# turbocast/HTS-train-WORLD

Measured on AMD Instinct MI355X. Metric: WORLD analysis+synthesis frames/sec @16kHz, 5ms hop, higher is better.
Workload: dtype f64

## Files before the change

### hts-train-world_amd/csrc/synthesis.hip

```cpp
#include <stdlib.h>

#include <algorithm>
#include <vector>

#include "batch.hpp"
#include "common.hpp"
#include "fastmath.hpp"
#include "fft.hpp"
#include "partition.hpp"

namespace wm {

__device__ __forceinline__ double coarse_f0(const double* __restrict__ f0, int nf, int j, double lowest) {
  if (j < nf) {
    const double v = f0[j];
    return v < lowest ? 0.0 : v;
  }
  const int j2 = nf >= 2 ? nf - 2 : nf - 1;
  const double a = f0[nf - 1] < lowest ? 0.0 : f0[nf - 1];
  const double b = f0[j2] < lowest ? 0.0 : f0[j2];
  return a * 2 - b;
}
__device__ __forceinline__ double coarse_vuv(const double* __restrict__ f0, int nf, int j, double lowest) {
  if (j < nf) return (f0[j] < lowest ? 0.0 : f0[j]) == 0.0 ? 0.0 : 1.0;
  const double a = (f0[nf - 1] < lowest ? 0.0 : f0[nf - 1]) == 0.0 ? 0.0 : 1.0;
  const int j2 = nf >= 2 ? nf - 2 : nf - 1;
  const double b = (f0[j2] < lowest ? 0.0 : f0[j2]) == 0.0 ? 0.0 : 1.0;
  return a * 2 - b;
}

#define WM_CHAIN_PRIO __builtin_amdgcn_s_setprio(3);
__global__ __launch_bounds__(256) void synth_inc_kernel(
    const int* __restrict__ utts, const double* __restrict__ f0, const int64_t* __restrict__ f_off,
    const int64_t* __restrict__ y_off, int fs, double fp, double lowest_f0, double* __restrict__ vuv_out,
    double* __restrict__ inc_out) {
#pragma clang fp contract(off)
  WM_CHAIN_PRIO
  const int u = utts[blockIdx.y];
  const double* f0u = f0 + f_off[u];
  const int nf = (int)(f_off[u + 1] - f_off[u]);
  const int64_t yb = y_off[u];
  const int ylen = (int)(y_off[u + 1] - yb);
  for (int i = blockIdx.x * 256 + threadIdx.x; i < ylen; i += gridDim.x * 256) {
    const double t = i / (double)fs;
    int kg = (int)(t / fp) + 1;
    if (kg > nf + 1) kg = nf + 1;
    if (kg < 0) kg = 0;
    while (kg <= nf && kg * fp <= t) ++kg;
    while (kg > 0 && (kg - 1) * fp > t) --kg;
    const int k = kg < 1 ? 1 : (kg > nf ? nf : kg);
    const double x0 = (k - 1) * fp, x1 = k * fp;
    const double h = x1 - x0;
    const double s = (t - x0) / h;
    const double fa = coarse_f0(f0u, nf, k - 1, lowest_f0), fb = coarse_f0(f0u, nf, k, lowest_f0);
    const double va = coarse_vuv(f0u, nf, k - 1, lowest_f0), vb = coarse_vuv(f0u, nf, k, lowest_f0);
    double fi = fa + s * (fb - fa);
    const double vi = va + s * (vb - va);
    const double vv = vi > 0.5 ? 1.0 : 0.0;
    fi = vv == 0.0 ? kDefaultF0 : fi;
    vuv_out[yb + i] = vv;
    inc_out[yb + i] = 2.0 * kPi * fi / fs;
  }
}

__global__ __launch_bounds__(64) void synth_timebase_kernel(const int* __restrict__ utts,
                                                            const int64_t* __restrict__ y_off, double* phase) {
#pragma clang fp contract(off)
  WM_CHAIN_PRIO
  const int u = utts[blockIdx.x], lane = threadIdx.x;
  const int64_t yb = y_off[u];
  const int ylen = (int)(y_off[u + 1] - yb);
  double carry = 0.0;
  constexpr int kSuper = 1024, kPer = kSuper / 64;
  __shared__ double ring[2 * kSuper];
  const double* p = phase + yb;
  double stage[kPer];
  auto request = [&](int s0) {
#pragma unroll
    for (int q = 0; q < kPer; ++q) {
      const int idx = s0 + 64 * q + lane;
      stage[q] = p[imin(idx, ylen - 1)];
    }
  };
  auto park = [&](int half) {
#pragma unroll
    for (int q = 0; q < kPer; ++q) ring[half * kSuper + 64 * q + lane] = stage[q];
  };
  request(0);
  park(0);
  request(kSuper);
  __syncthreads();
  double r[16];
#pragma unroll
  for (int q = 0; q < 16; ++q) r[q] = ring[q];
  for (int c0 = 0; c0 < ylen; c0 += 64) {
    const int i = c0 + lane;
    if ((c0 & (kSuper - 1)) == 0) {
      park(((c0 / kSuper) + 1) & 1);
      request(c0 + 2 * kSuper);
      __syncthreads();
    }
    double t = carry;
#pragma unroll
    for (int g = 0; g < 4; ++g) {
      double n[16];
      const int nb = (c0 + 16 * (g + 1)) & (2 * kSuper - 1);
#pragma unroll
      for (int q = 0; q < 16; ++q) n[q] = ring[nb + q];
#define WM_STEP(R) "v_add_f64 %[t], %[t], %[" #R "]\n\ts_lshl_b64 exec, exec, 1\n\t"
      asm volatile(
          "s_lshl_b64 exec, -1, %[sh]\n\t"
          WM_STEP(b0) WM_STEP(b1) WM_STEP(b2) WM_STEP(b3) WM_STEP(b4) WM_STEP(b5) WM_STEP(b6) WM_STEP(b7)
          WM_STEP(b8) WM_STEP(b9) WM_STEP(b10) WM_STEP(b11) WM_STEP(b12) WM_STEP(b13) WM_STEP(b14)
          "v_add_f64 %[t], %[t], %[b15]\n\t"
          "s_mov_b64 exec, -1"
          : [t] "+v"(t)
          : [sh] "n"(16 * g), [b0] "v"(r[0]), [b1] "v"(r[1]), [b2] "v"(r[2]), [b3] "v"(r[3]), [b4] "v"(r[4]),
            [b5] "v"(r[5]), [b6] "v"(r[6]), [b7] "v"(r[7]), [b8] "v"(r[8]), [b9] "v"(r[9]), [b10] "v"(r[10]),
            [b11] "v"(r[11]), [b12] "v"(r[12]), [b13] "v"(r[13]), [b14] "v"(r[14]), [b15] "v"(r[15])
          : "scc");
#undef WM_STEP
#pragma unroll
      for (int q = 0; q < 16; ++q) r[q] = n[q];
    }
    if (i < ylen) phase[yb + i] = t;
    carry = lane63(t);
  }
}

__device__ __forceinline__ double wrap_two_pi(double t) {
  const double two_pi = 2.0 * kPi;
  const double a = fabs(t);
  double kq = floor(a * (1.0 / two_pi));
  double w = __fma_rn(-kq, two_pi, a);
  if (w < 0.0) { kq -= 1.0; w = __fma_rn(-kq, two_pi, a); }
  if (w >= two_pi) { kq += 1.0; w = __fma_rn(-kq, two_pi, a); }
  return copysign(w, t);
}

constexpr int kSearchSub = 8, kSearchTile = 256 * kSearchSub;
template <bool WRITE>
__global__ __launch_bounds__(256) void synth_pulse_search_kernel(
    const int* __restrict__ utts, const int64_t* __restrict__ y_off, const double* __restrict__ phase, int fs,
    int tiles_max, int* __restrict__ tile_cnt, int* __restrict__ pulse_idx, double* __restrict__ pulse_shift,
    int* __restrict__ pulse_cnt) {
#pragma clang fp contract(off)
  WM_CHAIN_PRIO
  __shared__ int wave_cnt[kSearchSub][4];
  __shared__ int red[4];
  const int u = utts[blockIdx.y], tile = blockIdx.x;
  const int lane = threadIdx.x & 63, wv = threadIdx.x >> 6;
  const int64_t yb = y_off[u];
  const int ylen = (int)(y_off[u + 1] - yb);
  const int i0 = tile * kSearchTile;
  if (i0 >= ylen && !(WRITE && tile == 0)) return;
  int* cnt_u = tile_cnt + (int64_t)u * tiles_max;
  int count = 0;
  if (WRITE) {
    const int ntile = (ylen + kSearchTile - 1) / kSearchTile;
    int before = 0, all = 0;
    for (int j = threadIdx.x; j < ntile; j += 256) {
      const int c = cnt_u[j];
      all += c;
      if (j < tile) before += c;
    }
    before = wave_sum_i(before);
    all = wave_sum_i(all);
    if (lane == 0) red[wv] = before;
    __syncthreads();
    count = red[0] + red[1] + red[2] + red[3];
    __syncthreads();
    if (tile == 0) {
      if (lane == 0) red[wv] = all;
      __syncthreads();
      if (threadIdx.x == 0) pulse_cnt[u] = red[0] + red[1] + red[2] + red[3];
      __syncthreads();
    }
    if (i0 >= ylen) return;
  }
  double tc[kSearchSub], tp[kSearchSub];
#pragma unroll
  for (int q = 0; q < kSearchSub; ++q) {
    const int i = i0 + 256 * q + threadIdx.x;
    const bool in = i >= 1 && i < ylen;
    tc[q] = phase[yb + (in ? i : 0)];
    tp[q] = phase[yb + (in ? i - 1 : 0)];
  }
  bool hit[kSearchSub];
  double wrap[kSearchSub], prev[kSearchSub];
  unsigned long long bal[kSearchSub];
#pragma unroll
  for (int q = 0; q < kSearchSub; ++q) {
    const int i = i0 + 256 * q + threadIdx.x;
    wrap[q] = wrap_two_pi(tc[q]);
    prev[q] = wrap_two_pi(tp[q]);
    hit[q] = i >= 1 && i < ylen && fabs(wrap[q] - prev[q]) > kPi;
    bal[q] = __ballot(hit[q]);
    if (lane == 0) wave_cnt[q][wv] = __popcll(bal[q]);
  }
  __syncthreads();
  if (!WRITE) {
    if (threadIdx.x == 0) {
      int c = 0;
#pragma unroll
      for (int q = 0; q < kSearchSub; ++q) c += wave_cnt[q][0] + wave_cnt[q][1] + wave_cnt[q][2] + wave_cnt[q][3];
      cnt_u[tile] = c;
    }
    return;
  }
#pragma unroll
  for (int q = 0; q < kSearchSub; ++q) {
    const int i = i0 + 256 * q + threadIdx.x;
    int base = count;
    for (int w = 0; w < wv; ++w) base += wave_cnt[q][w];
    if (hit[q]) {
      const int dst = base + __popcll(bal[q] & ((1ull << lane) - 1ull));
      const double y1 = prev[q] - 2.0 * kPi, y2 = wrap[q];
      const double xx = -y1 / (y2 - y1);
      pulse_idx[yb + dst] = i - 1;
      pulse_shift[yb + dst] = xx / fs;
    }
    count += wave_cnt[q][0] + wave_cnt[q][1] + wave_cnt[q][2] + wave_cnt[q][3];
  }
}

__global__ __launch_bounds__(256) void synth_pulse_off_kernel(const int* __restrict__ utts, const int* __restrict__ cnt,
                                                              int n_list, int64_t base, int64_t* __restrict__ off,
                                                              int64_t* __restrict__ info) {
  __shared__ int64_t part[256];
  __shared__ int mx[256];
  const int per = (n_list + 255) / 256;
  const int lo = threadIdx.x * per, hi = imin(n_list, lo + per);
  int64_t sum = 0;
  int m = 0;
  for (int k = lo; k < hi; ++k) {
    const int c = cnt[utts[k]];
    sum += c;
    m = imax(m, c);
  }
  part[threadIdx.x] = sum;
  mx[threadIdx.x] = m;
  __syncthreads();
  if (threadIdx.x == 0) {
    int64_t run = 0;
    int mm = 0;
    for (int i = 0; i < 256; ++i) {
      const int64_t v = part[i];
      part[i] = run;
      run += v;
      mm = imax(mm, mx[i]);
    }
    info[0] = run;
    info[1] = mm;
    __threadfence_system();
  }
  __syncthreads();
  int64_t run = base + part[threadIdx.x];
  for (int k = lo; k < hi; ++k) {
    const int u = utts[k];
    off[u] = run;
    run += cnt[u];
  }
}

__global__ void synth_dc_remover_kernel(int fft_size, double* __restrict__ dcr) {
  if (threadIdx.x != 0 || blockIdx.x != 0) return;
  double dc = 0.0;
  const int h = fft_size / 2;
  for (int i = 0; i < h; ++i) {
    dcr[i] = 0.5 - 0.5 * cos(2.0 * kPi * (i + 1.0) / (1.0 + fft_size));
    dcr[fft_size - i - 1] = dcr[i];
    dc += dcr[i] * 2.0;
  }
  for (int i = 0; i < h; ++i) {
    dcr[i] /= dc;
    dcr[fft_size - i - 1] = dcr[i];
  }
}

__device__ __forceinline__ double safe_ap(double v) {
  const double m = 0.999999999999 < v ? 0.999999999999 : v;
  return 0.001 > m ? 0.001 : m;
}

template <int N>
__device__ __forceinline__ void minimum_phase(const double* ls, cpx* img, const FftTw<N>& tw, int lane,
                                              cpx (&mp)[N / 64 + 1]) {
  constexpr int M = N / 64, F = 2 * N, H = N;
  lane = opaque_lane(lane);
  cpx v[M];
#pragma unroll
  for (int m = 0; m < M; ++m) {
    const int i0 = 2 * (lane + 64 * m), i1 = i0 + 1;
    v[m] = make_double2(ls[i0 <= H ? i0 : F - i0], ls[i1 <= H ? i1 : F - i1]);
  }
  rfft_forward<N>(v, img, img, tw, lane);
#pragma unroll
  for (int m = 0; m < M; ++m) {
    const int i0 = 2 * (lane + 64 * m), i1 = i0 + 1;
    const double xa = img[imin(i0, H)].x, xb = img[imin(i1, H)].x;
    const double a = i0 <= H ? ((i0 == 0 || i0 == H) ? xa : 2.0 * xa) : 0.0;
    const double b = i1 < H ? 2.0 * xb : 0.0;
    v[m] = make_double2(a, b);
  }
  rfft_forward<N>(v, img, img, tw, lane);
#pragma unroll
  for (int m = 0; m <= M; ++m) {
    const int k = m < M ? lane + 64 * m : N;
    const cpx s = img[k];
    const double amp = wm_exp(s.x / F);
    double sn, cs;
    if (m < M) {
      sincospi(s.y * (1.0 / (kPi * F)), &sn, &cs);
    } else {
      sn = 0.0;
      cs = 1.0;
    }
    mp[m] = make_double2(amp * cs, amp * sn);
    __builtin_amdgcn_sched_barrier(0);
  }
  wave_sync();
}

template <int N>
__device__ __forceinline__ void minimum_phase_pair(const double* lsp, const double* lsa, cpx* img, const FftTw<N>& tw,
                                                   int lane, double (&php)[N / 64], double (&pha)[N / 64]) {
  constexpr int M = N / 64, F = 2 * N, H = N;
  static_assert(M >= 8 && M % 8 == 0, "the constant factors below are eighths of a half turn");
  lane = opaque_lane(lane);
  cpx v[M];
#pragma unroll
  for (int m = 0; m < M; ++m) {
    const int i0 = 2 * (lane + 64 * m), i1 = i0 + 1;
    const int a0 = i0 <= H ? i0 : F - i0, a1 = i1 <= H ? i1 : F - i1;
    const double p0 = lsp[a0], q0 = lsa[a0], p1 = lsp[a1], q1 = lsa[a1];
    v[m] = make_double2(p0 - q1, q0 + p1);
  }
  fft_forward<N>(v, img, tw, lane);
  auto turn = [&](int m, cpx e0, cpx& e, double& inv) {
    const int k64 = 32 * m / M;
    e = k64 % 16 == 0 ? e0 : cmul(e0, cconj(cis64(k64 % 16)));
    if (k64 / 16 == 1) e = make_double2(-e.y, e.x);
    const double r0 = __builtin_amdgcn_rcp(e.y);
    const double r1 = __builtin_fma(__builtin_fma(-e.y, r0, 1.0), r0, r0);
    inv = (m == 0 && lane == 0) ? 0.0 : 0.5 * r1;
  };
  wave_sync();
#pragma unroll
  for (int m = 0; m < M; ++m) img[lane + 64 * m] = v[m];
  wave_sync();
  {
    const cpx e0 = cconj(make_double2(opaque_d(tw.wsplit.x), opaque_d(tw.wsplit.y)));
    cpx zp[M];
#pragma unroll
    for (int m = 0; m < M; ++m) zp[m] = img[(N - (lane + 64 * m)) & (N - 1)];
    wave_sync();
#pragma unroll
    for (int m = 0; m < M; ++m) {
      cpx e;
      double inv;
      turn(m, e0, e, inv);
      const cpx R = make_double2((zp[m].x - v[m].x) * inv, (zp[m].y - v[m].y) * inv);
      const double ax = v[m].x + __builtin_fma(e.x, R.y, e.y * R.x) + R.x;
      const double ay = v[m].y - __builtin_fma(e.x, R.x, -(e.y * R.y)) + R.y;
      const cpx g = (m == 0 && lane == 0) ? make_double2(0.0, 0.0) : make_double2(2.0 * ax, 2.0 * ay);
      img[lane + 64 * m] = g;
      __builtin_amdgcn_sched_barrier(0);
    }
    if (lane == 0) img[H] = make_double2(0.0, 0.0);
  }
  wave_sync();
#pragma unroll
  for (int m = 0; m < M; ++m) {
    const int i0 = 2 * (lane + 64 * m), i1 = i0 + 1;
    const cpx c0 = img[i0 <= H ? i0 : F - i0], c1 = img[i1 <= H ? i1 : F - i1];
    const double s0 = i0 <= H ? 1.0 : -1.0, s1 = i1 <= H ? 1.0 : -1.0;
    v[m] = make_double2(s0 * c0.x - s1 * c1.y, s0 * c0.y + s1 * c1.x);
  }
  fft_forward<N>(v, img, tw, lane);
  wave_sync();
#pragma unroll
  for (int m = 0; m < M; ++m) img[lane + 64 * m] = v[m];
  wave_sync();
  {
    const cpx e0 = cconj(make_double2(opaque_d(tw.wsplit.x), opaque_d(tw.wsplit.y)));
#pragma unroll
    for (int m = 0; m < M; ++m) {
      const int k = lane + 64 * m;
      const cpx zp = img[(N - k) & (N - 1)];
      cpx e;
      double inv;
      turn(m, e0, e, inv);
      const cpx R = make_double2(-(zp.x + v[m].x) * inv, -(zp.y + v[m].y) * inv);
      const double gx = v[m].x + __builtin_fma(e.x, R.y, e.y * R.x) + R.x;
      const double gy = v[m].y - __builtin_fma(e.x, R.x, -(e.y * R.y)) + R.y;
      const bool zero = m == 0 && lane == 0;
      php[m] = zero ? 0.0 : gy * (0.5 / F);
      pha[m] = zero ? 0.0 : -gx * (0.5 / F);
      __builtin_amdgcn_sched_barrier(0);
    }
  }
  wave_sync();
}

struct PulseRec {
  int64_t fbase;
  int nf;
  int idx;
  int roff;
  int noise_size;
  double shift;
  double cvuv;
};

struct PulseVoicedPred {
  const PulseRec* rec;
  __device__ bool operator()(int i) const { return rec[i].cvuv > 0.5; }
};

constexpr int kOlaStep = 128;
__host__ __device__ inline int64_t ola_table_base(int64_t yb, int u) { return yb / kOlaStep + 2 * (int64_t)u; }

__global__ __launch_bounds__(256) void synth_pulse_rec_kernel(
    const int* __restrict__ utts, const int64_t* __restrict__ f_off, const int64_t* __restrict__ y_off,
    const int64_t* __restrict__ p_off, const int* __restrict__ p_cnt, const int* __restrict__ pulse_idx,
    const double* __restrict__ pulse_shift, const double* __restrict__ vuv, PulseRec* __restrict__ rec,
    int* __restrict__ first) {
  const int u = utts[blockIdx.y];
  const int64_t pb = p_off[u];
  const int np = p_cnt[u];
  const int64_t yb = y_off[u];
  const int ylen = (int)(y_off[u + 1] - yb);
  int* fu = first + ola_table_base(yb, u);
  const int m_last = (ylen + kOlaStep - 1) / kOlaStep;
  for (int pi = blockIdx.x * 256 + threadIdx.x; pi < np; pi += gridDim.x * 256) {
    PulseRec r;
    r.fbase = f_off[u];
    r.nf = (int)(f_off[u + 1] - f_off[u]);
    r.idx = pulse_idx[yb + pi];
    r.roff = r.idx - pulse_idx[yb];
    r.noise_size = pulse_idx[yb + imin(np - 1, pi + 1)] - r.idx;
    r.shift = pulse_shift[yb + pi];
    r.cvuv = vuv[yb + r.idx];
    rec[pb + pi] = r;
    const int prev = pi > 0 ? pulse_idx[yb + pi - 1] : -1;
    for (int m = prev < 0 ? 0 : prev / kOlaStep + 1; m <= imin(m_last, r.idx / kOlaStep); ++m) fu[m] = pi;
    if (pi == np - 1)
      for (int m = r.idx / kOlaStep + 1; m <= m_last; ++m) fu[m] = np;
  }
}

template <int F>
__global__ __launch_bounds__(64, F >= 4096 ? 1 : (F == 1024 ? 4 : (F < 1024 ? 3 : 2))) void synth_pulse_kernel(
    const double* __restrict__ sp, const double* __restrict__ ap, const PulseRec* __restrict__ rec,
    const double* __restrict__ dcr, const uint32_t* __restrict__ rtab, int fs, double fp, int64_t p_begin,
    int64_t p_end, const int* __restrict__ perm, double* __restrict__ resp) {
  constexpr int N = F / 2, M = N / 64, H = F / 2, MB = M + 1;
  constexpr bool LEAN = F == 2048 || F == 1024;
  constexpr bool PAIRED = F == 1024;
  __shared__ __attribute__((aligned(16))) double smem[2 * FftLds<N>::kElems + (LEAN ? 0 : H + 2)];
  cpx* img = reinterpret_cast<cpx*>(smem);
  double* ls = LEAN ? smem : smem + 2 * FftLds<N>::kElems;
  const int lane0 = threadIdx.x;
  FftTw<N> tw;
  tw.init(lane0);

  WM_FOR_EACH_LISTED(pi, perm, p_end - p_begin) {
    const int64_t p = p_begin + pi;
    const int lane = opaque_lane(lane0);
    const PulseRec r = rec[p];
    const int nf = r.nf;
    const int idx = r.idx;
    const int noise_size = r.noise_size;
    const double cvuv = r.cvuv;
    const double ctime = idx / (double)fs;
    const double shift = r.shift;

    const int ff = imin(nf - 1, (int)floor(ctime / fp));
    const int fc = imin(nf - 1, (int)ceil(ctime / fp));
    const double wgt = ff == fc ? 0.0 : ctime / fp - ff;
    const double* s0 = sp + (r.fbase + ff) * (int64_t)(H + 1);
    const double* s1 = sp + (r.fbase + fc) * (int64_t)(H + 1);
    const double* a0 = ap + (r.fbase + ff) * (int64_t)(H + 1);
    const double* a1 = ap + (r.fbase + fc) * (int64_t)(H + 1);
    auto spectral = [&](double (&env)[MB], double (&rat)[MB]) {
#pragma unroll
      for (int m = 0; m < MB; ++m) {
        const int k = m < M ? lane + 64 * m : H;
        env[m] = (1.0 - wgt) * fabs(s0[k]) + wgt * fabs(s1[k]);
        const double a = (1.0 - wgt) * safe_ap(a0[k]) + wgt * safe_ap(a1[k]);
        rat[m] = a * a;
      }
    };
    double env_keep[LEAN ? 1 : MB], rat_keep[LEAN ? 1 : MB];
    double rat0;
    if constexpr (LEAN) {
      const double a = (1.0 - wgt) * safe_ap(a0[0]) + wgt * safe_ap(a1[0]);
      rat0 = uniform_d(a * a);
    } else {
      spectral(env_keep, rat_keep);
      rat0 = __shfl(rat_keep[0], 0, 64);
    }
    double* out = resp + (p - p_begin) * (int64_t)F;

    double xp[LEAN ? 1 : M];
    double dc = 0.0;
    const bool periodic = !(cvuv <= 0.5 || rat0 > 0.999);
#pragma unroll
    for (int m = 0; m < (LEAN ? 1 : M); ++m) xp[m] = 0.0;
    if (periodic) {
      wave_sync();
      auto log_periodic = [&](const double (&env)[MB], const double (&rat)[MB]) {
#pragma unroll
        for (int m = 0; m < M; ++m) {
          ls[lane + 64 * m] = wm_log(env[m] * (1.0 - rat[m]) + kSafe) / 2.0;
          __builtin_amdgcn_sched_barrier(0);
        }
        if (lane == 0) ls[H] = wm_log(env[M] * (1.0 - rat[M]) + kSafe) / 2.0;
      };
      cpx mp[MB];
      if constexpr (PAIRED) {
        double* ls2 = ls + H + 2;
        {
          double env[MB], rat[MB];
          spectral(env, rat);
#pragma unroll
          for (int m = 0; m < MB; ++m) {
            const int k = m < M ? lane + 64 * m : H;
            const double lp = wm_log(env[m] * (1.0 - rat[m]) + kSafe) / 2.0;
            const double la = wm_log(env[m] * rat[m]) / 2.0;
            if (m < M || lane == 0) {
              ls[k] = lp;
              ls2[k] = la;
            }
            __builtin_amdgcn_sched_barrier(0);
          }
        }
        wave_sync();
        {
          double php[M], pha[M];
          minimum_phase_pair<N>(ls, ls2, img, tw, lane, php, pha);
#pragma unroll
          for (int m = 0; m < M; ++m) {
            out[lane + 64 * m] = pha[m];
            mp[m] = make_double2(0.0, php[m]);
          }
          mp[M] = make_double2(0.0, 0.0);
        }
        {
          double env[MB], rat[MB];
          spectral(env, rat);
#pragma unroll
          for (int m = 0; m < MB; ++m) mp[m].x = wm_sqrt(env[m] * (1.0 - rat[m]) + kSafe);
        }
#pragma unroll
        for (int m = 0; m < MB; ++m) {
          double sn = 0.0, cs = 1.0;
          if (m < M) sincospi(mp[m].y * (1.0 / kPi), &sn, &cs);
          mp[m] = make_double2(mp[m].x * cs, mp[m].x * sn);
          __builtin_amdgcn_sched_barrier(0);
        }
      } else {
        if constexpr (LEAN) {
          double env[MB], rat[MB];
          spectral(env, rat);
          log_periodic(env, rat);
        } else {
          log_periodic(env_keep, rat_keep);
        }
        wave_sync();
        minimum_phase<N>(ls, img, tw, lane, mp);
      }
      const double coef = 2.0 * kPi * shift * fs / F;
      double rc, rs, dc64, ds64;
      const double ch = coef * (1.0 / kPi);
      double snH, reH;
      wm_sincospi(ch * lane, &rs, &rc);
      wm_sincospi(ch * 64.0, &ds64, &dc64);
      wm_sincospi(ch * H, &snH, &reH);
#pragma unroll
      for (int m = 0; m < MB; ++m) {
        const int k = m < M ? lane + 64 * m : H;
        const double re2 = m < M ? rc : reH;
        {
          const double nc = rc * dc64 - rs * ds64;
          rs = rs * dc64 + rc * ds64;
          rc = nc;
        }
        const double im2 = wm_sqrt(1.0 - re2 * re2);
        const cpx s = make_double2(mp[m].x * re2 + mp[m].y * im2, mp[m].y * re2 - mp[m].x * im2);
        if (m < M || lane == 0) img[k] = s;
        __builtin_amdgcn_sched_barrier(0);
      }
      cpx v[M];
      rfft_backward<N>(img, v, img, tw, lane);
#pragma unroll
      for (int m = 0; m < M / 2; ++m) {
        if constexpr (LEAN) {
          const int i0 = 2 * (lane + 64 * m);
          *reinterpret_cast<cpx*>(out + i0 + H) = v[m];
        } else {
          xp[2 * m] = v[m].x;
          xp[2 * m + 1] = v[m].y;
        }
        dc += v[m].x + v[m].y;
      }
      dc = wave_sum(dc);
      if constexpr (LEAN) dc = uniform_d(dc);
      wave_sync();
    }

    wave_sync();
    cpx mp[MB];
    if (PAIRED && periodic) {
      {
        const int lp_ = opaque_lane(lane);
#pragma unroll
        for (int m = 0; m < M; ++m) mp[m] = make_double2(0.0, out[lp_ + 64 * m]);
        mp[M] = make_double2(0.0, 0.0);
      }
      {
        double env[MB], rat[MB];
        spectral(env, rat);
#pragma unroll
        for (int m = 0; m < MB; ++m) mp[m].x = wm_sqrt(env[m] * rat[m]);
      }
#pragma unroll
      for (int m = 0; m < MB; ++m) {
        double sn = 0.0, cs = 1.0;
        if (m < M) sincospi(mp[m].y * (1.0 / kPi), &sn, &cs);
        mp[m] = make_double2(mp[m].x * cs, mp[m].x * sn);
        __builtin_amdgcn_sched_barrier(0);
      }
    } else {
      {
        auto log_aperiodic = [&](const double (&env)[MB], const double (&rat)[MB]) {
#pragma unroll
          for (int m = 0; m < MB; ++m) {
            const int k = m < M ? lane + 64 * m : H;
            const double val = wm_log(cvuv != 0.0 ? env[m] * rat[m] : env[m]) / 2.0;
            if (m < M || lane == 0) ls[k] = val;
            __builtin_amdgcn_sched_barrier(0);
          }
        };
        if constexpr (LEAN) {
          double env[MB], rat[MB];
          spectral(env, rat);
          log_aperiodic(env, rat);
        } else {
          log_aperiodic(env_keep, rat_keep);
        }
      }
      wave_sync();
      minimum_phase<N>(ls, img, tw, lane, mp);
    }
    cpx v[M];
    {
      const int ln = LEAN ? opaque_lane(lane) : lane;
      const int roff = r.roff;
      double sum = 0.0;
#pragma unroll
      for (int m = 0; m < M; ++m) {
        const int i0 = 2 * (ln + 64 * m);
        const double n0 = i0 < noise_size ? randn_at(rtab, roff + i0) : 0.0;
        const double n1 = i0 + 1 < noise_size ? randn_at(rtab, roff + i0 + 1) : 0.0;
        v[m] = make_double2(n0, n1);
        sum += n0 + n1;
      }
      const double avg = wave_sum(sum) / noise_size;
#pragma unroll
      for (int m = 0; m < M; ++m) {
        const int i0 = 2 * (ln + 64 * m);
        if (i0 < noise_size) v[m].x -= avg;
        if (i0 + 1 < noise_size) v[m].y -= avg;
      }
    }
    rfft_forward_nz<N>(v, img, img, tw, lane, (noise_size + 127) >> 7);
#pragma unroll
    for (int m = 0; m < MB; ++m) {
      const int k = m < M ? lane + 64 * m : H;
      const cpx ns = img[k];
      const cpx s = make_double2(mp[m].x * ns.x - mp[m].y * ns.y, mp[m].x * ns.y + mp[m].y * ns.x);
      if (m < M || lane == 0) img[k] = s;
    }
    rfft_backward<N>(img, v, img, tw, lane);

    const double sq = sqrt((double)noise_size);
    cpx xq[LEAN ? M / 2 : 1];
    const int lo = LEAN ? opaque_lane(lane) : lane;
    if constexpr (LEAN) {
#pragma unroll
      for (int m = 0; m < M / 2; ++m)
        xq[m] = periodic ? *reinterpret_cast<const cpx*>(out + 2 * (lo + 64 * m) + H) : make_double2(0.0, 0.0);
    }
#pragma unroll
    for (int m = 0; m < M; ++m) {
      const int n = lo + 64 * m;
      const int i0 = 2 * n;
      double r0, r1;
      if (m < M / 2) {
        const double x0 = LEAN ? xq[LEAN ? m : 0].x : xp[LEAN ? 0 : 2 * m];
        const double x1 = LEAN ? xq[LEAN ? m : 0].y : xp[LEAN ? 0 : 2 * m + 1];
        const double2 dr = *reinterpret_cast<const double2*>(dcr + i0 + H);
        const double p0 = periodic ? x0 - dc * dr.x : 0.0;
        const double p1 = periodic ? x1 - dc * dr.y : 0.0;
        r0 = (p0 * sq + v[m].x) / F;
        r1 = (p1 * sq + v[m].y) / F;
        out[i0 + H] = r0;
        out[i0 + 1 + H] = r1;
      } else {
        const double2 dr = *reinterpret_cast<const double2*>(dcr + i0 - H);
        const double p0 = periodic ? -dc * dr.x : 0.0;
        const double p1 = periodic ? -dc * dr.y : 0.0;
        r0 = (p0 * sq + v[m].x) / F;
        r1 = (p1 * sq + v[m].y) / F;
        out[i0 - H] = r0;
        out[i0 + 1 - H] = r1;
      }
    }
    wave_sync();
  }
}

}
#include "synth_pulse_bp.hpp"
namespace wm {

constexpr int kOlaQ = 4, kOlaSeg = 128 * kOlaQ, kOlaWaves = 4;
__global__ __launch_bounds__(64 * kOlaWaves) void synth_ola_kernel(const int* __restrict__ utts,
                                                                   const int64_t* __restrict__ y_off,
                                                                   const int64_t* __restrict__ p_off,
                                                                   const int* __restrict__ p_cnt,
                                                                   const int* __restrict__ pulse_idx,
                                                                   const int* __restrict__ first, int fft_size,
                                                                   int64_t p_begin, int64_t p_end,
                                                                   const double* __restrict__ resp,
                                                                   double* __restrict__ y) {
  const int u = utts[blockIdx.y];
  const int lane = threadIdx.x & 63;
  const int64_t yb = y_off[u];
  const int ylen = (int)(y_off[u + 1] - yb);
  const int n0 = (blockIdx.x * kOlaWaves + (threadIdx.x >> 6)) * kOlaSeg;
  const int64_t pu = p_off[u];
  const int np = p_cnt[u];
  if (n0 >= ylen || np == 0 || pu >= p_end || pu + np <= p_begin) return;
  const int h = fft_size / 2;
  const int* fu = first + ola_table_base(yb, u);
  const int m_last = (ylen + kOlaStep - 1) / kOlaStep;
  const int lo_s = imax(0, n0 - h), hi_s = n0 + kOlaSeg + h - 2;
  int pa = fu[lo_s / kOlaStep];
  int pb = fu[imin(m_last, hi_s / kOlaStep + 1)];
  const int64_t rel_a = p_begin - pu, rel_b = p_end - pu;
  pa = rel_a > pa ? (int)(rel_a < np ? rel_a : np) : pa;
  pb = rel_b < pb ? (int)(rel_b > 0 ? rel_b : 0) : pb;
  if (pa >= pb) return;
  const int* pidx = pulse_idx + yb;
  double2_a8 acc[kOlaQ];
#pragma unroll
  for (int q = 0; q < kOlaQ; ++q) {
    const int n = n0 + 128 * q + 2 * lane;
    acc[q].x = n < ylen ? y[yb + n] : 0.0;
    acc[q].y = n + 1 < ylen ? y[yb + n + 1] : 0.0;
  }
  for (int base = pa; base < pb; base += 64) {
    const int cnt = imin(64, pb - base);
    const int my_idx = pidx[base + imin(lane, cnt - 1)];
    for (int k = 0; k < cnt; ++k) {
      const int idx = __builtin_amdgcn_readlane(my_idx, k);
      const int s = idx - h + 1 - n0;
      const double* row = resp + ((int64_t)(pu + base + k) - p_begin) * fft_size;
#pragma unroll
      for (int q = 0; q < kOlaQ; ++q) {
        const int c0 = 128 * q - s;
        if (c0 + 127 < 0 || c0 >= fft_size) continue;
        const int j = c0 + 2 * lane;
        if (c0 >= 0 && c0 + 127 < fft_size) {
          const double2_a8 v = *reinterpret_cast<const double2_a8*>(row + j);
          acc[q].x += v.x;
          acc[q].y += v.y;
        } else {
          const bool in0 = j >= 0 && j < fft_size, in1 = j + 1 >= 0 && j + 1 < fft_size;
          const double v0 = row[imin(fft_size - 1, imax(0, j))];
          const double v1 = row[imin(fft_size - 1, imax(0, j + 1))];
          if (in0) acc[q].x += v0;
          if (in1) acc[q].y += v1;
        }
      }
    }
  }
#pragma unroll
  for (int q = 0; q < kOlaQ; ++q) {
    const int n = n0 + 128 * q + 2 * lane;
    if (n < ylen) y[yb + n] = acc[q].x;
    if (n + 1 < ylen) y[yb + n + 1] = acc[q].y;
  }
}

struct SynPart {
  const int* d_list;
  int n;
  int max_y_len;
  int64_t p_base;
  int64_t total_p = 0;
  int max_np = 0;
};

struct SynWs : StageWs {
  int* d_pulse_idx = nullptr;
  double* d_pulse_shift = nullptr;
  double* d_vuv = nullptr;
  double* d_phase = nullptr;
  int* d_pulse_cnt = nullptr;
  int* d_pulse_tile_cnt = nullptr;
  int64_t* d_pulse_off = nullptr;
  int* d_pulse_first = nullptr;
  int* d_order = nullptr;
  std::vector<int> sorted;
  std::vector<int> order_host;
  const double* d_dc_remover = nullptr;
  PulseRec* d_pulse_rec = nullptr;
  int64_t pulse_rec_cap = 0;
  int* d_pulse_perm = nullptr;
  int64_t total_p = 0, chunk = 0;
  ~SynWs() override {
    dev_free(d_pulse_rec);
    dev_free(d_pulse_perm);
  }
};
static SynWs& syn_ws(Batch& b) { return static_cast<SynWs&>(*b.syn); }

static int synthesis_arena(Batch& b, hipStream_t st) {
  Context& c = *b.ctx;
  const int F = b.p.fft_size;
  if (b.syn) return WM_OK;
  const size_t ny = (size_t)b.total_y, nu = (size_t)b.n_utt;
  const size_t tiles = (size_t)((b.max_y_len + kSearchTile - 1) / kSearchTile + 1);
  size_t at = 0;
  auto take = [&](size_t bytes) { const size_t o = at; at = (at + (bytes ? bytes : 8) + 255) & ~(size_t)255; return o; };
  const size_t o_idx = take(4 * ny), o_shift = take(8 * ny), o_vuv = take(8 * ny), o_phase = take(8 * ny);
  const size_t o_cnt = take(4 * nu), o_tile = take(4 * nu * tiles), o_off = take(8 * (nu + 1));
  const size_t o_first = take(4 * (ny / kOlaStep + 2 * nu + 4));
  const size_t o_order = take(4 * 2 * nu);
  const Table* dcr = nullptr;
  int rc = c.table({kDcRemover, {(double)F}}, dcr, [&](Table& t) {
    int r = wm_check(t.alloc(&t.d[0], sizeof(double) * (size_t)F));
    if (r) return r;
    hipLaunchKernelGGL(synth_dc_remover_kernel, dim3(1), dim3(64), 0, st, F, (double*)t.d[0]);
    return wm_check(hipStreamSynchronize(st));
  });
  if (rc) return rc;
  std::unique_ptr<SynWs> W(new SynWs());
  unsigned char* base = nullptr;
  rc = wm_check(W->alloc(&base, at));
  if (rc) return rc;
  if (!c.pulse) {
    std::unique_ptr<PulseInfo> pi(new PulseInfo());
    rc = wm_check(hipHostMalloc((void**)&pi->h, sizeof(int64_t) * 2, hipHostMallocMapped));
    if (!rc) rc = wm_check(hipHostGetDevicePointer((void**)&pi->d, pi->h, 0));
    if (rc) return rc;
    c.pulse = std::move(pi);
  }
  W->d_pulse_idx = (int*)(base + o_idx); W->d_pulse_shift = (double*)(base + o_shift);
  W->d_vuv = (double*)(base + o_vuv); W->d_phase = (double*)(base + o_phase);
  W->d_pulse_cnt = (int*)(base + o_cnt); W->d_pulse_tile_cnt = (int*)(base + o_tile);
  W->d_pulse_off = (int64_t*)(base + o_off); W->d_dc_remover = (const double*)dcr->d[0];
  W->d_pulse_first = (int*)(base + o_first);
  W->d_order = (int*)(base + o_order);
  std::vector<int>& order = W->order_host;
  order.resize(2 * nu);
  for (size_t u = 0; u < nu; ++u) order[u] = order[nu + u] = (int)u;
  std::stable_sort(order.begin() + (long)nu, order.end(), [&](int x, int y) { return b.y_len[(size_t)x] < b.y_len[(size_t)y]; });
  W->sorted.assign(order.begin() + (long)nu, order.end());
  rc = wm_check(hipMemcpyAsync(W->d_order, order.data(), sizeof(int) * order.size(), hipMemcpyHostToDevice, st));
  if (rc) return rc;
  b.syn = std::move(W);
  return WM_OK;
}

static int synthesis_prepare_launch(Batch& b, hipStream_t st, const SynPart& part, const double* d_f0) {
  Context& c = *b.ctx;
  SynWs& W = syn_ws(b);
  const int F = b.p.fft_size, fs = b.p.fs;
  const double fp = b.p.frame_period / 1000.0;
  const double lowest_f0 = fs / F + 1.0;
  {
    const int tiles = imin(64, (part.max_y_len + 255) / 256);
    {
      TimedScope ts_(b.ctx, st, "synth_inc_kernel");
      hipLaunchKernelGGL(synth_inc_kernel, dim3(tiles, part.n), dim3(256), 0, st, part.d_list, d_f0, b.d_f_off,
                         b.d_y_off, fs, fp, lowest_f0, W.d_vuv, W.d_phase);
    }
    TimedScope ts_(b.ctx, st, "synth_timebase_kernel");
    hipLaunchKernelGGL(synth_timebase_kernel, dim3(part.n), dim3(64), 0, st, part.d_list, b.d_y_off, W.d_phase);
  }
  {
    TimedScope ts_(b.ctx, st, "synth_search_kernel");
    const int tiles_max = (b.max_y_len + kSearchTile - 1) / kSearchTile + 1;
    const int tiles_part = (part.max_y_len + kSearchTile - 1) / kSearchTile + 1;
    hipLaunchKernelGGL(synth_pulse_search_kernel<false>, dim3(tiles_part, part.n), dim3(256), 0, st, part.d_list,
                       b.d_y_off, W.d_phase, fs, tiles_max, W.d_pulse_tile_cnt, W.d_pulse_idx, W.d_pulse_shift,
                       W.d_pulse_cnt);
    hipLaunchKernelGGL(synth_pulse_search_kernel<true>, dim3(tiles_part, part.n), dim3(256), 0, st, part.d_list,
                       b.d_y_off, W.d_phase, fs, tiles_max, W.d_pulse_tile_cnt, W.d_pulse_idx, W.d_pulse_shift,
                       W.d_pulse_cnt);
  }
  hipLaunchKernelGGL(synth_pulse_off_kernel, dim3(1), dim3(256), 0, st, part.d_list, (const int*)W.d_pulse_cnt, part.n,
                     part.p_base, W.d_pulse_off, c.pulse->d);
  return wm_check(hipGetLastError());
}

static int synthesis_prepare_finish(Batch& b, hipStream_t st, SynPart& part, int64_t expect_more, bool in_flight) {
  Context& c = *b.ctx;
  SynWs& W = syn_ws(b);
  const int F = b.p.fft_size;
  part.total_p = c.pulse->h[0];
  part.max_np = (int)c.pulse->h[1];
  if (part.total_p == 0) return WM_OK;
  int64_t cap_mb = 4096;
  if (const char* e = getenv("WORLD_MI355_SCRATCH_MB")) cap_mb = atoll(e) > 0 ? atoll(e) : cap_mb;
  int64_t chunk = (cap_mb * 1024 * 1024 / 8) / F / 2;
  if (chunk < 1) chunk = 1;
  constexpr int pieces = 2;
  const int64_t list = part.total_p > expect_more ? part.total_p : expect_more;
  const int64_t share = (list + pieces - 1) / pieces;
  if (share >= 16384 && chunk > share) chunk = share;
  if (chunk > list) chunk = list;
  int rc = c.ensure_side();
  if (rc) return rc;
  if (in_flight) {
    chunk = W.chunk > 0 ? W.chunk : chunk;
  } else {
    rc = c.ensure_scratch((chunk < list || expect_more > 0 ? 2 : 1) * chunk * F, st);
    if (rc) return rc;
    W.chunk = chunk;
  }
  const int64_t need = part.p_base + part.total_p + (in_flight ? 0 : expect_more);
  if (need > W.pulse_rec_cap) {
    if (in_flight) {
      rc = wm_check(hipDeviceSynchronize());
      if (rc) return rc;
    }
    if (W.d_pulse_rec) dev_free(W.d_pulse_rec);
    W.d_pulse_rec = nullptr;
    W.pulse_rec_cap = 0;
    if (W.d_pulse_perm) dev_free(W.d_pulse_perm);
    W.d_pulse_perm = nullptr;
    const int64_t cap = need + need / 8 + 64;
    rc = wm_check(dev_alloc(&W.d_pulse_rec, sizeof(PulseRec) * (size_t)cap));
    if (rc) return rc;
    rc = wm_check(dev_alloc(&W.d_pulse_perm, sizeof(int) * (size_t)(cap + 2 * (cap / kPartBlock + 8))));
    if (rc) return rc;
    W.pulse_rec_cap = cap;
  }
  hipLaunchKernelGGL(synth_pulse_rec_kernel, dim3(imin(64, (part.max_np + 255) / 256), part.n), dim3(256), 0, st,
                     part.d_list, b.d_f_off, b.d_y_off, W.d_pulse_off, (const int*)W.d_pulse_cnt, W.d_pulse_idx,
                     W.d_pulse_shift, W.d_vuv, W.d_pulse_rec, W.d_pulse_first);
  const int64_t piece = W.chunk, p_end = part.p_base + part.total_p;
  int* part_scratch = W.d_pulse_perm + W.pulse_rec_cap + (in_flight ? W.pulse_rec_cap / kPartBlock + 8 : 0);
  for (int64_t p0 = part.p_base; p0 < p_end; p0 += piece) {
    const int64_t np = p_end - p0 < piece ? p_end - p0 : piece;
    launch_partition(st, PulseVoicedPred{W.d_pulse_rec + p0}, (int)np, part_scratch + 4,
                     W.d_pulse_perm + p0, part_scratch);
  }
  return wm_check(hipGetLastError());
}

static int synthesis_render_part(Batch& b, hipStream_t st, const SynPart& part, const double* d_sp, const double* d_ap,
                                 double* d_y, int& piece) {
  Context& c = *b.ctx;
  const SideStreams& s = *c.fork;
  SynWs& W = syn_ws(b);
  const int F = b.p.fft_size, fs = b.p.fs;
  const double fp = b.p.frame_period / 1000.0;
  const int64_t chunk = W.chunk;
  const int ola_tiles = (part.max_y_len + kOlaSeg * kOlaWaves - 1) / (kOlaSeg * kOlaWaves);
  int rc = WM_OK;
  const int64_t lo = part.p_base, hi = part.p_base + part.total_p;
  for (int64_t p0 = lo; p0 < hi && !rc; p0 += chunk, ++piece) {
    const int64_t p1 = p0 + chunk < hi ? p0 + chunk : hi;
    const int64_t np = p1 - p0;
    const int h = piece & 1;
    double* resp = c.d_scratch + (int64_t)h * chunk * F;
    const int grid = (int)(np < (int64_t)c.frame_grid ? np : (int64_t)c.frame_grid);
    if (piece >= 2) rc = wm_check(hipStreamWaitEvent(st, s.ev_ola[h], 0));
    if (rc) break;
#define WM_SY_CASE(FF, KERNEL)                                                                                  \
  case FF: {                                                                                                    \
    const int per_ = persistent_grid(c, KERNEL<FF>, 64, (int64_t)1 << 40);                               \
    hipLaunchKernelGGL(KERNEL<FF>, dim3(imin(grid, per_)), dim3(64), 0, st, d_sp, d_ap,                         \
                       W.d_pulse_rec, W.d_dc_remover, c.d_rng, fs, fp, p0, p1,                 \
                       (const int*)W.d_pulse_perm + p0, resp);                                                  \
  } break;
    {
      TimedScope ts_(b.ctx, st, "synth_pulse_kernel");
      switch (F) {
        WM_SY_CASE(512, synth_pulse_kernel)
        WM_SY_CASE(1024, synth_pulse_kernel)
        WM_SY_CASE(2048, synth_pulse_bp_kernel)
        WM_SY_CASE(4096, synth_pulse_kernel)
      }
    }
#undef WM_SY_CASE
    hipStream_t so = s.side;
    rc = wm_check(hipEventRecord(s.ev_pulse[h], st));
    rc = rc ? rc : wm_check(hipStreamWaitEvent(so, s.ev_pulse[h], 0));
    if (rc) break;
    {
      TimedScope ts2_(b.ctx, so, "synth_ola_kernel");
      hipLaunchKernelGGL(synth_ola_kernel, dim3(ola_tiles, part.n), dim3(64 * kOlaWaves), 0, so, part.d_list, b.d_y_off,
                         W.d_pulse_off, (const int*)W.d_pulse_cnt, W.d_pulse_idx, (const int*)W.d_pulse_first, F, p0,
                         p1, resp, d_y);
    }
    rc = wm_check(hipEventRecord(s.ev_ola[h], so));
  }
  return rc ? rc : wm_check(hipGetLastError());
}

static int synthesis_join(Batch& b, hipStream_t st, int pieces) {
  if (pieces == 0) return WM_OK;
  return wm_check(hipStreamWaitEvent(st, b.ctx->fork->ev_ola[(pieces - 1) & 1], 0));
}

static int synthesis_setup(Batch& b, hipStream_t st, double* d_y) {
  const int F = b.p.fft_size;
  if (F != 512 && F != 1024 && F != 2048 && F != 4096) return WM_ERR_UNSUPPORTED_FFT;
  int rc = b.ctx->ensure_rng(b.rng_bound_synthesis(), st);
  rc = rc ? rc : synthesis_arena(b, st);
  return rc ? rc : wm_check(hipMemsetAsync(d_y, 0, sizeof(double) * (size_t)b.total_y, st));
}

int synthesis_begin(Batch& b, hipStream_t st, const double* d_f0, double* d_y) {
  const int rc = synthesis_setup(b, st, d_y);
  if (rc) return rc;
  SynPart part{syn_ws(b).d_order, b.n_utt, b.max_y_len, 0};
  return synthesis_prepare_launch(b, st, part, d_f0);
}
int synthesis_prepare_wait(Batch& b, hipStream_t st) {
  SynWs& W = syn_ws(b);
  SynPart part{W.d_order, b.n_utt, b.max_y_len, 0};
  int rc = wm_check(hipStreamSynchronize(st));
  W.chunk = 0;
  rc = rc ? rc : synthesis_prepare_finish(b, st, part, 0, false);
  W.total_p = part.total_p;
  return rc;
}
int synthesis_prepare(Batch& b, hipStream_t st, const double* d_f0, double* d_y) {
  int rc = synthesis_begin(b, st, d_f0, d_y);
  return rc ? rc : synthesis_prepare_wait(b, st);
}

int synthesis_render(Batch& b, hipStream_t st, const double* d_sp, const double* d_ap, double* d_y) {
  const SynWs& W = syn_ws(b);
  if (W.total_p == 0) return WM_OK;
  SynPart part{W.d_order, b.n_utt, b.max_y_len, 0};
  part.total_p = W.total_p;
  int piece = 0;
  int rc = synthesis_render_part(b, st, part, d_sp, d_ap, d_y, piece);
  return rc ? rc : synthesis_join(b, st, piece);
}

int launch_synthesis(Batch& b, const double* d_f0, const double* d_sp, const double* d_ap, double* d_y) {
  Context& c = *b.ctx;
  const hipStream_t st = c.stream;
  if (b.n_utt < 16 || b.total_y < (int64_t)4 << 20) {
    int rc = synthesis_prepare(b, st, d_f0, d_y);
    return rc ? rc : synthesis_render(b, st, d_sp, d_ap, d_y);
  }
  int rc = synthesis_setup(b, st, d_y);
  rc = rc ? rc : c.ensure_side();
  rc = rc ? rc : c.ensure_split();
  if (rc) return rc;
  SynWs& W = syn_ws(b);
  const SplitStreams& s = *c.split;
  int n_a = 0;
  int64_t acc = 0;
  while (n_a < b.n_utt - 1 && acc < b.total_y / 3) acc += b.y_len[(size_t)W.sorted[(size_t)n_a++]];
  const int* sorted = W.d_order + b.n_utt;
  SynPart pa{sorted, n_a, b.y_len[(size_t)W.sorted[(size_t)n_a - 1]], 0};
  SynPart pb{sorted + n_a, b.n_utt - n_a, b.max_y_len, 0};
  rc = wm_check(hipEventRecord(s.ev_call, st));
  rc = rc ? rc : synthesis_prepare_launch(b, st, pa, d_f0);
  rc = rc ? rc : wm_check(hipStreamSynchronize(st));
  if (rc) return rc;
  W.chunk = 0;
  const int64_t guess_b = (int64_t)((double)c.pulse->h[0] * (double)(b.total_y - acc) / (double)(acc > 0 ? acc : 1) * 1.25) + 1024;
  rc = synthesis_prepare_finish(b, st, pa, guess_b, false);
  if (rc) return rc;
  pb.p_base = pa.total_p;
  rc = wm_check(hipStreamWaitEvent(s.prep, s.ev_call, 0));
  rc = rc ? rc : synthesis_prepare_launch(b, s.prep, pb, d_f0);
  int piece = 0;
  if (!rc && pa.total_p > 0) rc = synthesis_render_part(b, st, pa, d_sp, d_ap, d_y, piece);
  rc = rc ? rc : wm_check(hipStreamSynchronize(s.prep));
  if (rc) return rc;
  rc = synthesis_prepare_finish(b, s.prep, pb, 0, pa.total_p > 0);
  rc = rc ? rc : wm_check(hipEventRecord(s.ev_prep_b, s.prep));
  rc = rc ? rc : wm_check(hipStreamWaitEvent(st, s.ev_prep_b, 0));
  if (!rc && pb.total_p > 0) rc = synthesis_render_part(b, st, pb, d_sp, d_ap, d_y, piece);
  W.total_p = pa.total_p + pb.total_p;
  return rc ? rc : synthesis_join(b, st, piece);
}

#ifdef WM_PHASE
int phase_read_synthesis(unsigned long long* out32) { return wm_phase_read(out32); }
#endif

}
```

Before: 22.20 million.

## Compute minimum-phase amplitude directly and use half-zero FFT for phase only

Replaces the minimum-phase routine with a version that returns only the phase (in turns). The amplitude is now the square root of the already-known power spectrum rather than exp of a cepstral FFT result. The second FFT gets a half-zero input hint (NZM), so the transform can skip work on the zero upper half. It also skips the aperiodicity load for unvoiced pulses in the lean path and adds compile-time phase-timing instrumentation macros. The direct amplitude should match the exp-of-cepstrum result up to rounding, but that equivalence depends on the cepstrum being exact.

```diff
diff --git a/hts-train-world_amd/csrc/synthesis.hip b/hts-train-world_amd/csrc/synthesis.hip
--- a/hts-train-world_amd/csrc/synthesis.hip
+++ b/hts-train-world_amd/csrc/synthesis.hip
@@ -284,9 +284,10 @@
 }
 
 template <int N>
-__device__ __forceinline__ void minimum_phase(const double* ls, cpx* img, const FftTw<N>& tw, int lane,
-                                              cpx (&mp)[N / 64 + 1]) {
+__device__ __forceinline__ void minimum_phase_turns(const double* ls, cpx* img, const FftTw<N>& tw, int lane,
+                                                    double (&pht)[N / 64]) {
   constexpr int M = N / 64, F = 2 * N, H = N;
+  constexpr int NZM = N < 512 ? M : M / 2;
   lane = opaque_lane(lane);
   cpx v[M];
 #pragma unroll
@@ -296,30 +297,23 @@
   }
   rfft_forward<N>(v, img, img, tw, lane);
 #pragma unroll
-  for (int m = 0; m < M; ++m) {
-    const int i0 = 2 * (lane + 64 * m), i1 = i0 + 1;
-    const double xa = img[imin(i0, H)].x, xb = img[imin(i1, H)].x;
-    const double a = i0 <= H ? ((i0 == 0 || i0 == H) ? xa : 2.0 * xa) : 0.0;
-    const double b = i1 < H ? 2.0 * xb : 0.0;
-    v[m] = make_double2(a, b);
-  }
-  rfft_forward<N>(v, img, img, tw, lane);
-#pragma unroll
-  for (int m = 0; m <= M; ++m) {
-    const int k = m < M ? lane + 64 * m : N;
-    const cpx s = img[k];
-    const double amp = wm_exp(s.x / F);
-    double sn, cs;
-    if (m < M) {
-      sincospi(s.y * (1.0 / (kPi * F)), &sn, &cs);
-    } else {
-      sn = 0.0;
-      cs = 1.0;
-    }
-    mp[m] = make_double2(amp * cs, amp * sn);
-    __builtin_amdgcn_sched_barrier(0);
-  }
+  for (int m = 0; m < M / 2; ++m) {
+    const int i0 = 2 * (lane + 64 * m);
+    const double xa = img[i0].x, xb = img[i0 + 1].x;
+    v[m] = make_double2(i0 == 0 ? 0.0 : 2.0 * xa, 2.0 * xb);
+  }
+#pragma unroll
+  for (int m = M / 2; m < M; ++m) v[m] = make_double2(0.0, 0.0);
+  rfft_forward<N, NZM>(v, img, img, tw, lane);
+#pragma unroll
+  for (int m = 0; m < M; ++m) pht[m] = img[lane + 64 * m].y * (1.0 / (kPi * F));
   wave_sync();
+}
+
+__device__ __forceinline__ cpx polar_turns(double amp, double pht) {
+  double sn, cs;
+  sincospi(pht, &sn, &cs);
+  return make_double2(amp * cs, amp * sn);
 }
 
 template <int N>
@@ -450,6 +444,14 @@
   }
 }
 
+#ifdef WM_PHASE
+#define WM_PHASE_MARK_BY(cond, k_true, k_false) if (cond) { WM_PHASE_MARK(k_true) } else { WM_PHASE_MARK(k_false) }
+#define WM_PHASE_COUNT_BY(cond, k_true, k_false) if (cond) { phase_clock_.acc[k_true] += 1; } else { phase_clock_.acc[k_false] += 1; }
+#else
+#define WM_PHASE_MARK_BY(cond, k_true, k_false)
+#define WM_PHASE_COUNT_BY(cond, k_true, k_false)
+#endif
+
 template <int F>
 __global__ __launch_bounds__(64, F >= 4096 ? 1 : (F == 1024 ? 4 : (F < 1024 ? 3 : 2))) void synth_pulse_kernel(
     const double* __restrict__ sp, const double* __restrict__ ap, const PulseRec* __restrict__ rec,
@@ -465,7 +467,9 @@
   FftTw<N> tw;
   tw.init(lane0);
 
+  WM_PHASE_DECL
   WM_FOR_EACH_LISTED(pi, perm, p_end - p_begin) {
+    WM_PHASE_MARK(0)
     const int64_t p = p_begin + pi;
     const int lane = opaque_lane(lane0);
     const PulseRec r = rec[p];
@@ -492,11 +496,21 @@
         rat[m] = a * a;
       }
     };
+    auto envelope = [&](double (&env)[MB]) {
+#pragma unroll
+      for (int m = 0; m < MB; ++m) {
+        const int k = m < M ? lane + 64 * m : H;
+        env[m] = (1.0 - wgt) * fabs(s0[k]) + wgt * fabs(s1[k]);
+      }
+    };
     double env_keep[LEAN ? 1 : MB], rat_keep[LEAN ? 1 : MB];
     double rat0;
     if constexpr (LEAN) {
-      const double a = (1.0 - wgt) * safe_ap(a0[0]) + wgt * safe_ap(a1[0]);
-      rat0 = uniform_d(a * a);
+      rat0 = 1.0;
+      if (!(cvuv <= 0.5)) {
+        const double a = (1.0 - wgt) * safe_ap(a0[0]) + wgt * safe_ap(a1[0]);
+        rat0 = uniform_d(a * a);
+      }
     } else {
       spectral(env_keep, rat_keep);
       rat0 = __shfl(rat_keep[0], 0, 64);
@@ -508,6 +522,8 @@
     const bool periodic = !(cvuv <= 0.5 || rat0 > 0.999);
 #pragma unroll
     for (int m = 0; m < (LEAN ? 1 : M); ++m) xp[m] = 0.0;
+    WM_PHASE_COUNT_BY(periodic, 13, 14)
+    WM_PHASE_MARK(1)
     if (periodic) {
       wave_sync();
       auto log_periodic = [&](const double (&env)[MB], const double (&rat)[MB]) {
@@ -537,9 +553,11 @@
           }
         }
         wave_sync();
+        WM_PHASE_MARK(2)
         {
           double php[M], pha[M];
           minimum_phase_pair<N>(ls, ls2, img, tw, lane, php, pha);
+          WM_PHASE_MARK(3)
 #pragma unroll
           for (int m = 0; m < M; ++m) {
             out[lane + 64 * m] = pha[m];
@@ -569,7 +587,25 @@
           log_periodic(env_keep, rat_keep);
         }
         wave_sync();
-        minimum_phase<N>(ls, img, tw, lane, mp);
+        WM_PHASE_MARK(2)
+        double pht[M];
+        minimum_phase_turns<N>(ls, img, tw, lane, pht);
+        WM_PHASE_MARK(3)
+        auto polar_periodic = [&](const double (&env)[MB], const double (&rat)[MB]) {
+#pragma unroll
+          for (int m = 0; m < MB; ++m) {
+            const double amp = wm_sqrt(env[m] * (1.0 - rat[m]) + kSafe);
+            mp[m] = m < M ? polar_turns(amp, pht[m < M ? m : 0]) : make_double2(amp, 0.0);
+            __builtin_amdgcn_sched_barrier(0);
+          }
+        };
+        if constexpr (LEAN) {
+          double env[MB], rat[MB];
+          spectral(env, rat);
+          polar_periodic(env, rat);
+        } else {
+          polar_periodic(env_keep, rat_keep);
+        }
       }
       const double coef = 2.0 * kPi * shift * fs / F;
       double rc, rs, dc64, ds64;
@@ -608,6 +644,7 @@
       dc = wave_sum(dc);
       if constexpr (LEAN) dc = uniform_d(dc);
       wave_sync();
+      WM_PHASE_MARK(4)
     }
 
     wave_sync();
@@ -633,27 +670,43 @@
         __builtin_amdgcn_sched_barrier(0);
       }
     } else {
-      {
-        auto log_aperiodic = [&](const double (&env)[MB], const double (&rat)[MB]) {
-#pragma unroll
-          for (int m = 0; m < MB; ++m) {
-            const int k = m < M ? lane + 64 * m : H;
-            const double val = wm_log(cvuv != 0.0 ? env[m] * rat[m] : env[m]) / 2.0;
-            if (m < M || lane == 0) ls[k] = val;
-            __builtin_amdgcn_sched_barrier(0);
+      auto aperiodic_power = [&](double (&pwr)[MB]) {
+        if constexpr (LEAN) {
+          if (cvuv != 0.0) {
+            double rat[MB];
+            spectral(pwr, rat);
+#pragma unroll
+            for (int m = 0; m < MB; ++m) pwr[m] *= rat[m];
+          } else {
+            envelope(pwr);
           }
-        };
-        if constexpr (LEAN) {
-          double env[MB], rat[MB];
-          spectral(env, rat);
-          log_aperiodic(env, rat);
         } else {
-          log_aperiodic(env_keep, rat_keep);
+#pragma unroll
+          for (int m = 0; m < MB; ++m) pwr[m] = cvuv != 0.0 ? env_keep[m] * rat_keep[m] : env_keep[m];
         }
+      };
+      double pwr[MB];
+      aperiodic_power(pwr);
+#pragma unroll
+      for (int m = 0; m < MB; ++m) {
+        const int k = m < M ? lane + 64 * m : H;
+        const double val = wm_log(pwr[m]) / 2.0;
+        if (m < M || lane == 0) ls[k] = val;
+        __builtin_amdgcn_sched_barrier(0);
       }
       wave_sync();
-      minimum_phase<N>(ls, img, tw, lane, mp);
-    }
+      WM_PHASE_MARK_BY(periodic, 5, 8)
+      double pht[M];
+      minimum_phase_turns<N>(ls, img, tw, lane, pht);
+      WM_PHASE_MARK_BY(periodic, 6, 9)
+#pragma unroll
+      for (int m = 0; m < MB; ++m) {
+        const double amp = wm_sqrt(pwr[m]);
+        mp[m] = m < M ? polar_turns(amp, pht[m < M ? m : 0]) : make_double2(amp, 0.0);
+        __builtin_amdgcn_sched_barrier(0);
+      }
+    }
+    WM_PHASE_MARK_BY(periodic, 7, 10)
     cpx v[M];
     {
       const int ln = LEAN ? opaque_lane(lane) : lane;
@@ -719,7 +772,9 @@
       }
     }
     wave_sync();
-  }
+    WM_PHASE_MARK_BY(periodic, 12, 11)
+  }
+  WM_PHASE_FLUSH(0)
 }
 
 }
```

Measured after the change: 22.61 million, median of 6. 1.8% higher.
